# Hendrik1704/GPBayesTools-HIC

Hardware: AMD Instinct MI355X
Metric: MCMC steps/s x walkers (walker log-posterior evaluations per second, whole job) (higher is better)
Workload: dtype f64

## Files before the change

gpbayestools_hic_amd/csrc/gpb_api.hip:

```cpp
#include "gpb_internal.h"
#include <dlfcn.h>
#include <math.h>
#include <string.h>
#include <vector>
#include <mutex>
#include <condition_variable>

using namespace gpb;

namespace {

template <typename T>
int dev_alloc(gpb_ctx* ctx, T** p, int64_t count) {
    if (*p) {
        if (ctx->side_stream) GPB_HIP(hipStreamSynchronize(ctx->side_stream));
        pool_free(*p); *p = nullptr;
    }
    GPB_HIP(pool_malloc(reinterpret_cast<void**>(p), sizeof(T) * (size_t)(count > 0 ? count : 1)));
    return 0;
}
template <typename T>
void dev_free(T** p) {
    if (*p) { pool_free(*p); *p = nullptr; }
}
// ... 1008 lines not shown
}

extern "C" int gpb_ctx_option(gpb_ctx* ctx, int key, int value) {
    if (!ctx) return GPB_E_ARG;
#ifndef GPB_DEBUG_VARIANTS
    if ((key == 26 && value != 0) || (key == 32 && value != 0))
        GPB_FAIL(GPB_E_ARG, "gpb_ctx_option: this value selects a hook of the debug build only");
#endif
    switch (key) {
        case 0: if (value < -1 || value > 1) return GPB_E_ARG; ctx->force_xcd = value; break;
        case 4: if (value < 0 || value % 64) return GPB_E_ARG; ctx->chol_outer = value; break;
        case 5: if (value < 1 || value > 3) return GPB_E_ARG; ctx->resident_order = value; break;
        case 7: if (value < 0) return GPB_E_ARG; ctx->narrow_switch = value; break;
        case 8: if (value < 0) return GPB_E_ARG; ctx->mvn_wg_switch = value; break;
        case 9: if (value != 64 && value != 128) return GPB_E_ARG; ctx->chol_inner_tile = value; break;
        case 10: if (value < 0 || value > 1) return GPB_E_ARG; ctx->tile_priority = value; break;
        case 17: if (value < 0 || value > 1) return GPB_E_ARG; ctx->tri_skip = value; break;
        case 18:
            if (value < 0 || value > 2) return GPB_E_ARG;
            ctx->kcross_dot = value;
            if (ctx->have_theta) {
                const int rc = choose_forms(ctx);
                if (rc) return rc;
            }
            break;
        case 19: if (value < 0 || value > 64) return GPB_E_ARG; ctx->kcross_chunks = value; break;
        case 20: if (value < 1 || value > 2) return GPB_E_ARG; ctx->kcross_wpl = value; break;
        case 23: if (value < 0 || value > 1) return GPB_E_ARG; ctx->lowrank = value; break;
        case 22: if (value < 0) return GPB_E_ARG; ctx->mid_switch = value; break;
        case 11: if (value < 0 || value > 1) return GPB_E_ARG; ctx->fuse_finalize = value; break;
        case 12: if (value != 0 && value != 64 && value != 128) return GPB_E_ARG; ctx->trtri_tile = value; break;
        case 14: if (value != 0 && value != 64 && value != 128) return GPB_E_ARG; ctx->syrk_tile = value; break;
        case 25: if (value < 0 || value > 1) return GPB_E_ARG; ctx->chol_lookahead = value; break;
        case 26: if (value < 0 || value > 64) return GPB_E_ARG; ctx->sim_ranks = value; break;
        case 27: if (value < 0 || value > 1) return GPB_E_ARG; ctx->compact = value; break;
        case 28: if (value < 0 || value > 1) return GPB_E_ARG; ctx->tile_by_live = value; break;
        case 29: if (value < 0 || value > 2) return GPB_E_ARG; ctx->premark = value; break;
        case 30: if (value < 0 || value > 1) return GPB_E_ARG; ctx->fuse_accept_propose = value; break;
        case 32: if (value < 0 || value > 63) return GPB_E_ARG; ctx->sim_rank = value; break;
        case 36: if (value < 0 || value > 2) return GPB_E_ARG; ctx->balance_shards = value; break;
        case 40: if (value < 0 || value > 1) return GPB_E_ARG; ctx->chain_batch = value; break;
        case 42:
            if (value != 0 && value != 32 && value != 64 && value != 65 && value != 128) return GPB_E_ARG;
            ctx->force_tile = value;
            break;
        case 43: if (value < 0 || value > 1) return GPB_E_ARG; ctx->force_generic_mvn = value != 0; break;
        case 47: if (value < 0 || value > 2) return GPB_E_ARG; ctx->chol_pair = value; break;
        case 49: if (value < 0 || value > 1) return GPB_E_ARG; ctx->lr_split = value; break;
        case 50: if (value != 0 && value != 64 && value != 128) return GPB_E_ARG; ctx->kinv_tile = value; break;
        case 51:
            if (value < 0 || value > 3) return GPB_E_ARG;
            ctx->predict_sliced = value;
            break;
        case 44: if (value < 0) return GPB_E_ARG; ctx->tile_switch = value > 0 ? value : 960; break;
        case 33: if (value < 0) return GPB_E_ARG; ctx->tile_switch_c = value; break;
        case 34: if (value < 0) return GPB_E_ARG; ctx->mid_switch_c = value; break;
        case 35: if (value < 0) return GPB_E_ARG; ctx->narrow_switch_c = value; break;
        default: return GPB_E_ARG;
    }
    return 0;
}

extern "C" int gpb_profile_fit_piece(gpb_ctx* ctx, int piece) {
    if (!ctx) return GPB_E_ARG;
    if (!ctx->have_theta) GPB_FAIL(GPB_E_STATE, "gpb_profile_fit_piece before gpb_gp_set_theta");
    GPB_HIP(hipSetDevice(ctx->device));
    ctx->factored = false;
    switch (piece) {
        case 0: return launch_kmat(ctx);
        case 1: return launch_potrf(ctx);
        case 2: return launch_trtri(ctx);
        case 3: return launch_alpha(ctx);
        default: return GPB_E_ARG;
    }
}



extern "C" int gpb_profile_enable(gpb_ctx* ctx, int on) {
    if (!ctx) return GPB_E_ARG;
    ctx->profile = on != 0;
    return 0;
}

extern "C" int gpb_profile_read(gpb_ctx* ctx, int64_t* launches, double* total_ms, double* units) {
    if (!ctx || !launches || !total_ms || !units) return GPB_E_ARG;
    GPB_HIP(hipSetDevice(ctx->device));
    GPB_HIP(hipStreamSynchronize(ctx->stream));
    double ms = 0.0;
    for (auto& ev : ctx->prof_events) {
        float t = 0.f;
        GPB_HIP(hipEventElapsedTime(&t, ev.first, ev.second));
        ms += t;
        (void)hipEventDestroy(ev.first);
        (void)hipEventDestroy(ev.second);
    }
    if (ctx->prof_compacted) {
        unsigned long long live = 0;
        GPB_HIP(hipMemcpy(&live, ctx->rows_live, sizeof(live), hipMemcpyDeviceToHost));
        GPB_HIP(hipMemset(ctx->rows_live, 0, sizeof(live)));
        ctx->prof_units += (ctx->prof_gps > 0.0 ? ctx->prof_gps : (double)ctx->P) * (double)live;
        ctx->prof_compacted = false;
    }
    *launches = (int64_t)ctx->prof_events.size();
    *total_ms = ms;
    *units = ctx->prof_units;
// ... 42 lines not shown
```

gpbayestools_hic_amd/csrc/gpb_internal.h:

```cpp
#pragma once
#include <hip/hip_runtime.h>
#include <stdint.h>
#include <string>
#include <utility>
#include <vector>
#include "../../include/gpbayes.h"
#include "../../include/gpbayes_debug.h"

namespace gpb {

constexpr int NB = 64;
constexpr int WPAD = 128;
constexpr int KX_CHUNK = 64;
constexpr int MAX_D = 64;

inline int64_t round_up(int64_t a, int64_t b) { return (a + b - 1) / b * b; }
__host__ __device__ inline int64_t imin64(int64_t a, int64_t b) { return a < b ? a : b; }

}

struct GpSel {
    const int* map;
    const int* n;
    int N;
    int64_t x_stride, xm_stride;
    __device__ __forceinline__ int q(int a) const { return map ? map[a] : a; }
    __device__ __forceinline__ int64_t Nq(int qq) const { return n ? (int64_t)n[qq] : (int64_t)N; }
};

__host__ __device__ __forceinline__ int64_t pad_front(int64_t Np, int64_t N) { return ((Np - N) / 16) * 16; }

struct LoopGroup;
struct gpb_ctx {
    int device = 0;
    hipStream_t stream = nullptr;
    bool own_stream = false;
    std::string err;

    int64_t N = 0, Np = 0, d = 0, dpad = 0, P = 0;
    int kind = 0;
    double alpha_reg = 0.0;
    bool have_theta = false, factored = false;
    double* h_theta = nullptr;
    bool multi = false;
    int64_t Pstore = 0;
    int* gpN = nullptr;
    int* gpmap = nullptr;
    bool subset = false;
    std::vector<int> h_N;
    std::vector<int> h_map;
    GpSel sel() const {
        return GpSel{subset ? gpmap : nullptr, multi ? gpN : nullptr, (int)N, multi ? Np * dpad : 0, multi ? dpad : 0};
    }
    double* X = nullptr;
    double* Xsc = nullptr;
    double* xmean = nullptr;
    double* muS = nullptr;
    double* Xc = nullptr;
    double* dnorm = nullptr;
    std::vector<double> h_ext;
    std::vector<int> h_form;
    int* gpform = nullptr;
    int* kmtiles = nullptr;
    int n_diff = 0;
    double gram_limit = 1024.0;
    double* ls = nullptr;
    double* amp = nullptr;
    double* noise = nullptr;
    double* Z = nullptr;
    double* K = nullptr;
    double* Linv = nullptr;
    int predict_sliced = 3;
    int8_t* slA = nullptr;
    int8_t* slB = nullptr;
    double* sl_scale = nullptr;
    bool slA_valid = false;
    int slA_depth = 0;
    int64_t slB_cap = 0;
    int batch_sliced = 0;
    bool want_kst = false;
    double* T = nullptr;
    double* yv = nullptr;
    double* alpha = nullptr;
    double* apart = nullptr;
    int* info = nullptr;
    double* lmlbuf = nullptr;
    double* gpart = nullptr;
    int64_t gpart_cap = 0;

    int64_t Wcap = 0;
    int64_t last_W = 0;
    int64_t Wld = 0;
    double* Xs = nullptr;
    double* estd = nullptr;
    double* KsT = nullptr;
    double* mpart = nullptr;
    double* spart = nullptr;
    double* mean_pc = nullptr;
    double* var_pc = nullptr;
    unsigned long long* live_hint = nullptr;
    gpb_ctx* hint_from = nullptr;
    int fuse_accept_propose = 1;
    int balance_shards = 0;
    int* bal_ws = nullptr;
    int64_t bal_cap = 0;
    int sim_rank = 0;
    int tile_by_live = 1;
    int premark = 2;
    double* cmp_X = nullptr;
    int64_t cmp_X_cap = 0;
    int* cmp_idx = nullptr;
    int compact = 1;
    unsigned long long* rows_live = nullptr;
    bool prof_compacted = false;
    double* vbuf = nullptr;
    int64_t vbuf_cap = 0;
    double* gbuf = nullptr;
    int64_t gbuf_cap = 0;
    double* covbuf = nullptr;
    int64_t covbuf_cap = 0;
    double* out_stage = nullptr;
    int64_t out_cap = 0;
    int* cv_ws = nullptr;
    int64_t cv_cap = 0;
    std::vector<int> h_cv;
// ... 171 lines not shown
```

gpbayestools_hic_amd/csrc/gpb_sliced.hip:

```cpp
#include "gpb_internal.h"

namespace gpb {

typedef int v4i __attribute__((ext_vector_type(4)));
typedef int v16i __attribute__((ext_vector_type(16)));
typedef __attribute__((address_space(3))) void* sl_lds_ptr;

template <int D>
struct SlDig {
    static constexpr int LOW = D - 1, NLEV = 2 * D - 1 - LOW, BITS = 8 * D - 1;
    static constexpr unsigned long long HALF = 0x8080808080808080ull >> (64 - 8 * D);
};
constexpr int SL_DMAX = 7;
constexpr int64_t SL_NP_MAX = 16384;
constexpr int SL_BM = 128;
template <int D, int WTN>
struct SlGeo {
    static constexpr int BN = 64 * WTN;
    static constexpr int A_CHUNKS = D * 2 * (SL_BM / 64), B_CHUNKS = D * 2 * WTN, CHUNKS = A_CHUNKS + B_CHUNKS;
    static constexpr int STAGE = CHUNKS * 1024, NSTAGE = 3;
    static constexpr int LDS = NSTAGE * STAGE + SL_BM * 8;
    static constexpr int NPW = (CHUNKS + 7) / 8, REM = CHUNKS % 8;
};
constexpr int SL_RG = 8, SL_CG = 4;
constexpr double SL_RULE = 128.0;

template <int D>
__device__ __forceinline__ unsigned long long sl_digits(long long a) {
    return ((unsigned long long)a + SlDig<D>::HALF) ^ SlDig<D>::HALF;
}

__device__ __forceinline__ int sl_exponent(double m) {
    int ex;
    const double f = frexp(m, &ex);
    return f <= 0.99 ? ex : ex + 1;
}

__global__ __launch_bounds__(256) void k_sl_rowscale(const double* __restrict__ Linv, const double* __restrict__ amp,
                                                     double* __restrict__ rowscale, int* __restrict__ rowexp,
                                                     double* __restrict__ colscale, int64_t Np, int64_t Np128) {
    const int p = blockIdx.y, lane = threadIdx.x & 63;
    const int64_t j = (int64_t)blockIdx.x * 4 + (threadIdx.x >> 6);
    if (j >= Np128) return;
    double m = 0.0;
    if (j < Np) {
        const double* row = Linv + ((int64_t)p * Np + j) * Np;
        for (int64_t k = lane; k <= j; k += 64) m = fmax(m, fabs(row[k]));
#pragma unroll
        for (int o = 32; o > 0; o >>= 1) m = fmax(m, __shfl_xor(m, o));
    }
    if (lane == 0) {
        const int e = m > 0.0 ? sl_exponent(m) : 0;
        rowexp[(int64_t)p * Np128 + j] = e;
        rowscale[(int64_t)p * Np128 + j] = ldexp(1.0, e - 14);
        if (j == 0) colscale[p] = ldexp(1.0, sl_exponent(amp[p]));
    }
}

template <int D>
__global__ __launch_bounds__(256) void k_sl_slice_linv(const double* __restrict__ Linv, const int* __restrict__ rowexp,
                                                       int8_t* __restrict__ planes, int64_t Np, int64_t Np128) {
    const int p = blockIdx.z;
    const int64_t j = (int64_t)blockIdx.x * 256 + threadIdx.x, kb = blockIdx.y;
    if (j >= Np || kb * 16 > j) return;
    const double* src = Linv + ((int64_t)p * Np + j) * Np + kb * 16;
    const int e = rowexp[(int64_t)p * Np128 + j];
    unsigned long long dg[16];
#pragma unroll
    for (int i = 0; i < 16; ++i) {
        const double x = (kb * 16 + i <= j) ? src[i] : 0.0;
        dg[i] = sl_digits<D>(__double2ll_rn(ldexp(x, SlDig<D>::BITS - e)));
    }
    const int64_t plane = (Np / 16) * Np128 * 16;
    int8_t* dst = planes + (int64_t)p * D * plane + (kb * Np128 + j) * 16;
#pragma unroll
    for (int t = 0; t < D; ++t) {
// ... 23 lines not shown
        const int t = cb / (2 * per), q = (cb / per) & 1, h = cb % per;
        const int64_t ld = is_a ? Np128 : Wld, off = is_a ? mb : nb;
        const int8_t* plane = is_a ? Ap + t * a_plane : Bp + t * b_plane;
        const int8_t* src = plane + ((kb0 + q) * ld + off + 64 * h + lane) * 16;
        __builtin_amdgcn_global_load_lds((const void*)src, (sl_lds_ptr)(base + ch * 1024), 16, 0, 0);
    }
}

template <int N>
__device__ __forceinline__ void sl_wait_vm() { asm volatile("s_waitcnt vmcnt(%0)" ::"n"(N) : "memory"); }

template <int D, int WTN>
__device__ __forceinline__ void sl_wait_stage(bool more, bool full_count) {
    typedef SlGeo<D, WTN> G;
    if (!more) sl_wait_vm<0>();
    else if (full_count) sl_wait_vm<G::NPW>();
    else sl_wait_vm<G::NPW - 1>();
}

template <int D, int WTN>
__device__ __forceinline__ void sl_mma_step(const char* lds, int buf, int wm, int wn, int lane, v16i (&acc)[SlDig<D>::NLEV][WTN]) {
    typedef SlGeo<D, WTN> G;
    constexpr int LOW = SlDig<D>::LOW;
    const char* base = lds + buf * G::STAGE;
    const int q = lane >> 5, r = lane & 31;
    v4i a[D];
#pragma unroll
    for (int t = 0; t < D; ++t) a[t] = *reinterpret_cast<const v4i*>(base + ((t * 2 + q) * SL_BM + wm * 32 + r) * 16);
#pragma unroll
    for (int j = 0; j < WTN; ++j) {
        v4i b[D];
#pragma unroll
        for (int t = 0; t < D; ++t)
            b[t] = *reinterpret_cast<const v4i*>(base + G::A_CHUNKS * 1024 + ((t * 2 + q) * G::BN + wn * 32 * WTN + 32 * j + r) * 16);
#pragma unroll
        for (int tb = 0; tb < D; ++tb)
#pragma unroll
            for (int ta = 0; ta < D; ++ta) {
                if (ta + tb < LOW) continue;
                acc[ta + tb - LOW][j] = __builtin_amdgcn_mfma_i32_32x32x32_i8(a[ta], b[tb], acc[ta + tb - LOW][j], 0, 0, 0);
            }
    }
}

struct SlGP {
    const int8_t *A, *B;
    const double *rowscale, *colscale;
    double* spart;
    int P, p;
};
constexpr int SL_MAX_GP = GPB_MAX_MULTI_GP;
struct SlTable { SlGP gp[SL_MAX_GP]; };

template <int D, int WTN, bool MULTI>
__device__ __forceinline__ void predict_sliced_body(const SlGP& G0, const SlTable* __restrict__ tab, int64_t Np, int64_t Np128, int64_t Wld,
                                                    int P, int nI, int nW, int kskip, const int* __restrict__ nrows) {
    typedef SlGeo<D, WTN> G;
    constexpr int NLEV = SlDig<D>::NLEV;
    extern __shared__ __attribute__((aligned(16))) char lds[];
    if (nrows) nW = (*nrows + G::BN - 1) / G::BN;
    const int nG = (nI + SL_RG - 1) / SL_RG, nWG = (nW + SL_CG - 1) / SL_CG;
    const unsigned label = blockIdx.x & 7u, m = blockIdx.x >> 3;
    const unsigned sb = (m / (SL_RG * SL_CG)) * 8u + label, local = m % (SL_RG * SL_CG);
    if (sb >= (unsigned)(nG * P * nWG)) return;
    const int g = (int)(sb / (unsigned)(P * nWG)), rem = (int)(sb % (unsigned)(P * nWG));
    const int pg = rem / nWG, wg = rem % nWG;
    const SlGP gp = MULTI ? tab->gp[pg] : G0;
    const int p = MULTI ? gp.p : pg;
    const int8_t* __restrict__ A = gp.A;
    const int8_t* __restrict__ B = gp.B;
    const double* __restrict__ rowscale = gp.rowscale;
    const double* __restrict__ colscale = gp.colscale;
    double* __restrict__ spart = gp.spart;
    const int Pc = MULTI ? gp.P : P;
    const int ib = (nG - 1 - g) * SL_RG + (SL_RG - 1 - (int)(local / SL_CG)), wt = wg * SL_CG + (int)(local % SL_CG);
    if (ib >= nI || wt >= nW) return;
    const int tid = threadIdx.x, lane = tid & 63;
    const int wave = __builtin_amdgcn_readfirstlane(tid >> 6);
    const int wm = wave >> 1, wn = wave & 1;
    const int64_t mb = (int64_t)ib * SL_BM, nb = (int64_t)wt * G::BN;
    const bool fullc = G::REM == 0 || wave < G::REM;
    const int64_t a_plane = (Np / 16) * Np128 * 16, b_plane = (Np / 16) * Wld * 16;
    const int8_t* Ap = A + (int64_t)p * D * a_plane;
    const int8_t* Bp = B + (int64_t)p * D * b_plane;
    double* rs = reinterpret_cast<double*>(lds + G::NSTAGE * G::STAGE);
    if (tid < SL_BM) rs[tid] = rowscale[(int64_t)p * Np128 + mb + tid];
    const int64_t k_end = imin64(mb + SL_BM, Np);
    const int64_t ks = (kskip / 32) * 32;
    const int64_t k_begin = ks <= mb ? ks : 0;
    const int nsteps = (int)((k_end - k_begin) / 32);
    const int64_t kb_first = k_begin / 16;
    v16i acc[NLEV][WTN];
#pragma unroll
    for (int l = 0; l < NLEV; ++l)
#pragma unroll
        for (int j = 0; j < WTN; ++j)
#pragma unroll
            for (int r = 0; r < 16; ++r) acc[l][j][r] = 0;
    sl_dma_stage<D, WTN>(lds, 0, Ap, Bp, a_plane, b_plane, Np128, Wld, mb, nb, kb_first, wave, lane);
    if (nsteps > 1) sl_dma_stage<D, WTN>(lds, 1, Ap, Bp, a_plane, b_plane, Np128, Wld, mb, nb, kb_first + 2, wave, lane);
    for (int s = 0; s < nsteps; ++s) {
        asm volatile("s_waitcnt lgkmcnt(0)" ::: "memory");
        sl_wait_stage<D, WTN>(s + 1 < nsteps, fullc);
        __builtin_amdgcn_s_barrier();
        sl_mma_step<D, WTN>(lds, s % 3, wm, wn, lane, acc);
        if (s + 2 < nsteps)
            sl_dma_stage<D, WTN>(lds, (s + 2) % 3, Ap, Bp, a_plane, b_plane, Np128, Wld, mb, nb, kb_first + 2 * (int64_t)(s + 2), wave, lane);
    }
    asm volatile("s_waitcnt lgkmcnt(0)" ::: "memory");
    __builtin_amdgcn_s_barrier();
    const double cs = colscale[p];
    double* hand = reinterpret_cast<double*>(lds);
    double sums[WTN];
#pragma unroll
    for (int j = 0; j < WTN; ++j) {
        double sum = 0.0;
#pragma unroll
        for (int r = 0; r < 16; ++r) {
            double t = (double)acc[0][j][r];
#pragma unroll
            for (int l = 1; l < NLEV; ++l) t = fma(t, 1.0 / 256.0, (double)acc[l][j][r]);
            const int row = wm * 32 + (r & 3) + 8 * (r >> 2) + 4 * (lane >> 5);
            const double v = t * rs[row] * cs;
            sum = fma(v, v, sum);
        }
        sum += __shfl_xor(sum, 32);
        sums[j] = sum;
        if ((wm & 1) && lane < 32) hand[(wave * WTN + j) * 32 + lane] = sum;
    }
    __syncthreads();
    const int64_t blk = (int64_t)ib * 2 + (wm >> 1);
    if (!(wm & 1) && lane < 32 && blk * 64 < Np) {
#pragma unroll
        for (int j = 0; j < WTN; ++j)
            spart[(blk * Pc + p) * Wld + nb + wn * 32 * WTN + 32 * j + lane] = sums[j] + hand[((wave + 2) * WTN + j) * 32 + lane];
    }
}

template <int D, int WTN>
__global__ __launch_bounds__(512, 2) void k_predict_sliced(const SlGP gp, int64_t Np, int64_t Np128, int64_t Wld, int P, int nI, int nW,
                                                           int kskip, const int* __restrict__ nrows) {
    predict_sliced_body<D, WTN, false>(gp, nullptr, Np, Np128, Wld, P, nI, nW, kskip, nrows);
}

template <int D, int WTN>
__global__ __launch_bounds__(512, 2) void k_predict_sliced_multi(const SlTable tab, int64_t Np, int64_t Np128, int64_t Wld, int P, int nI,
                                                                 int nW, int kskip, const int* __restrict__ nrows) {
    predict_sliced_body<D, WTN, true>(tab.gp[0], &tab, Np, Np128, Wld, P, nI, nW, kskip, nrows);
}

int sliced_applies(const gpb_ctx* ctx) {
    if (!ctx->predict_sliced || ctx->multi || !ctx->h_theta || !ctx->have_theta) return 0;
    if (ctx->tile_trace) return 0;
    if (ctx->Np > SL_NP_MAX) return 0;
    if (ctx->predict_sliced == 3) return 7;
    if (ctx->predict_sliced == 2) return 6;
    const int64_t stride = ctx->d + 2;
    for (int64_t p = 0; p < ctx->P; ++p) {
        const double lc = ctx->h_theta[p * stride], ln = ctx->h_theta[p * stride + ctx->d + 1];
        if (!(1.0 + exp(lc - ln) <= SL_RULE)) return 0;
    }
    return 6;
}

void sliced_free(gpb_ctx* ctx) {
    if (ctx->slA) { pool_free(ctx->slA); ctx->slA = nullptr; }
    if (ctx->slB) { pool_free(ctx->slB); ctx->slB = nullptr; }
    if (ctx->sl_scale) { pool_free(ctx->sl_scale); ctx->sl_scale = nullptr; }
    ctx->slA_valid = false;
    ctx->slA_depth = 0;
    ctx->slB_cap = 0;
}

const double* sliced_colscale(const gpb_ctx* ctx) {
    return reinterpret_cast<const double*>(ctx->sl_scale) + ctx->P * round_up(ctx->Np, 128);
}

int sliced_prepare(gpb_ctx* ctx, int depth) {
    if (depth != 6 && depth != 7) GPB_FAIL(GPB_E_STATE, "gpb: internal: sliced_prepare at a depth other than 6 or 7");
    const int64_t Np = ctx->Np, Np128 = round_up(Np, 128), P = ctx->P;
    const size_t a_bytes = (size_t)P * SL_DMAX * (size_t)Np * (size_t)Np128;
    if (!ctx->slA) {
        GPB_HIP(pool_malloc_t(&ctx->slA, a_bytes));
        GPB_HIP(hipMemsetAsync(ctx->slA, 0, a_bytes, ctx->stream));
        GPB_HIP(pool_malloc_t(&ctx->sl_scale, sizeof(double) * (size_t)(P * Np128 + P) + sizeof(int) * (size_t)(P * Np128)));
        ctx->slA_valid = false;
    }
    double* rowscale = reinterpret_cast<double*>(ctx->sl_scale);
    double* colscale = rowscale + P * Np128;
    int* rowexp = reinterpret_cast<int*>(colscale + P);
    if (!ctx->slA_valid || ctx->slA_depth != depth) {
        hipLaunchKernelGGL(k_sl_rowscale, dim3((unsigned)((Np128 + 3) / 4), (unsigned)P), dim3(256), 0, ctx->stream, ctx->Linv,
                           ctx->amp, rowscale, rowexp, colscale, Np, Np128);
        const dim3 grid((unsigned)((Np + 255) / 256), (unsigned)(Np / 16), (unsigned)P);
        if (depth == 7)
            hipLaunchKernelGGL(k_sl_slice_linv<7>, grid, dim3(256), 0, ctx->stream, ctx->Linv, rowexp, ctx->slA, Np, Np128);
        else
            hipLaunchKernelGGL(k_sl_slice_linv<6>, grid, dim3(256), 0, ctx->stream, ctx->Linv, rowexp, ctx->slA, Np, Np128);
        ctx->slA_valid = true;
        ctx->slA_depth = depth;
    }
    if (ctx->slB_cap < ctx->Wcap || !ctx->slB) {
        if (ctx->slB) { GPB_HIP(hipStreamSynchronize(ctx->stream)); pool_free(ctx->slB); ctx->slB = nullptr; }
        GPB_HIP(pool_malloc_t(&ctx->slB, (size_t)P * SL_DMAX * (size_t)Np * (size_t)ctx->Wcap));
        ctx->slB_cap = ctx->Wcap;
    }
    GPB_HIP(hipGetLastError());
    return 0;
}

int sliced_read_kstar(gpb_ctx* ctx, int64_t p, int64_t pad, int64_t N, int64_t W, double* out) {
    const int D = ctx->batch_sliced;
    if (D != 6 && D != 7) GPB_FAIL(GPB_E_STATE, "gpb: internal: sliced_read_kstar without a sliced batch");
    const int64_t Np = ctx->Np, Wld = ctx->Wld, plane = (Np / 16) * Wld * 16;
    std::vector<int8_t> h((size_t)(D * plane));
    double cs = 0.0;
    GPB_HIP(hipStreamSynchronize(ctx->stream));
    GPB_HIP(hipMemcpy(h.data(), ctx->slB + p * D * plane, (size_t)(D * plane), hipMemcpyDeviceToHost));
    GPB_HIP(hipMemcpy(&cs, sliced_colscale(ctx) + p, sizeof(double), hipMemcpyDeviceToHost));
    for (int64_t n = 0; n < N; ++n)
        for (int64_t w = 0; w < W; ++w) {
            const int64_t k = pad + n;
            long long a = 0;
            for (int t = D - 1; t >= 0; --t) a = a * 256 + (long long)h[(size_t)(t * plane + ((k / 16) * Wld + w) * 16 + k % 16)];
            out[n * W + w] = ldexp((double)a, -(8 * D - 1)) * cs;
        }
    return 0;
}

static int sliced_wtn(const gpb_ctx* ctx, int depth, int64_t gps, int nI, int64_t W, const int* nrows_dev) {
    if (depth == 7) return 1;
    const int64_t Wsel = imin64(ctx->Wld, live_rows_estimate(ctx, W, nrows_dev, ctx->Wld));
    const int64_t tiles128 = gps * nI * ((Wsel + 127) / 128);
    int wtn = tiles128 >= 3 * (int64_t)ctx->num_cu ? 2 : 1;
    if (ctx->force_tile == 128) wtn = 2;
    if (ctx->force_tile == 64 || ctx->force_tile == 32 || ctx->force_tile == 65) wtn = 1;
    return wtn;
}

template <int D, int WTN, bool MULTI, class Arg>
static int sliced_launch(gpb_ctx* ctx, const Arg& arg, int64_t Np, int64_t Np128, int64_t Wld, int G, int nI, int kskip,
                         const int* nrows_dev) {
    typedef SlGeo<D, WTN> Geo;
    const int nW = (int)(Wld / Geo::BN);
    const int nG = (nI + SL_RG - 1) / SL_RG, nWG = (nW + SL_CG - 1) / SL_CG;
    const int64_t nSB = (int64_t)nG * G * nWG;
    const unsigned grid = (unsigned)(((nSB + 7) / 8) * 8 * SL_RG * SL_CG);
    if constexpr (MULTI) {
        GPB_HIP(hipFuncSetAttribute((const void*)k_predict_sliced_multi<D, WTN>, hipFuncAttributeMaxDynamicSharedMemorySize, Geo::LDS));
        hipLaunchKernelGGL((k_predict_sliced_multi<D, WTN>), dim3(grid), dim3(512), Geo::LDS, ctx->stream, arg, Np, Np128, Wld, G, nI, nW,
                           kskip, nrows_dev);
    } else {
        GPB_HIP(hipFuncSetAttribute((const void*)k_predict_sliced<D, WTN>, hipFuncAttributeMaxDynamicSharedMemorySize, Geo::LDS));
        hipLaunchKernelGGL((k_predict_sliced<D, WTN>), dim3(grid), dim3(512), Geo::LDS, ctx->stream, arg, Np, Np128, Wld, G, nI, nW,
                           kskip, nrows_dev);
    }
    return 0;
}

template <bool MULTI, class Arg>
static int sliced_dispatch(gpb_ctx* ctx, int depth, int wtn, const Arg& arg, int64_t Np, int64_t Np128, int64_t Wld, int G, int nI,
                           int kskip, const int* nrows_dev) {
    if (depth == 7) return sliced_launch<7, 1, MULTI>(ctx, arg, Np, Np128, Wld, G, nI, kskip, nrows_dev);
    if (wtn == 2) return sliced_launch<6, 2, MULTI>(ctx, arg, Np, Np128, Wld, G, nI, kskip, nrows_dev);
    return sliced_launch<6, 1, MULTI>(ctx, arg, Np, Np128, Wld, G, nI, kskip, nrows_dev);
}

int launch_vsq_sliced(gpb_ctx* ctx, int64_t W, const int* nrows_dev, int kskip) {
    const int64_t Np = ctx->Np, Np128 = round_up(Np, 128), P = ctx->P, Wld = ctx->Wld;
    const int depth = ctx->batch_sliced;
    if (!ctx->slA || !ctx->slA_valid || !ctx->slB || ctx->slA_depth != depth)
        GPB_FAIL(GPB_E_STATE, "gpb: internal: launch_vsq_sliced before sliced_prepare");
    const double* rowscale = reinterpret_cast<const double*>(ctx->sl_scale);
    const double* colscale = rowscale + P * Np128;
    const int nI = (int)(Np128 / SL_BM);
    const int wtn = sliced_wtn(ctx, depth, P, nI, W, nrows_dev);
    const SlGP gp{ctx->slA, ctx->slB, rowscale, colscale, ctx->spart, (int)P, 0};
    return sliced_dispatch<false>(ctx, depth, wtn, gp, Np, Np128, Wld, (int)P, nI, kskip, nrows_dev);
}

int launch_vsq_sliced_multi(gpb_ctx* const* ctxs, int E, int64_t W, const int* nrows_dev, int kskip) {
    gpb_ctx* ctx = ctxs[0];
    const int64_t Np = ctx->Np, Np128 = round_up(Np, 128), Wld = ctx->Wld;
    const int depth = ctx->batch_sliced;
    SlTable tab;
    int G = 0;
    for (int e = 0; e < E; ++e) {
        gpb_ctx* c = ctxs[e];
        if (!c->slA || !c->slA_valid || !c->slB || c->Np != Np || c->Wld != Wld || c->batch_sliced != depth || c->slA_depth != depth)
            GPB_FAIL(GPB_E_STATE, "gpb: internal: launch_vsq_sliced_multi over a context that is not prepared");
        const double* rowscale = reinterpret_cast<const double*>(c->sl_scale);
        const double* colscale = rowscale + c->P * Np128;
        for (int p = 0; p < (int)c->P; ++p, ++G) {
            if (G >= SL_MAX_GP) GPB_FAIL(GPB_E_STATE, "gpb: internal: launch_vsq_sliced_multi: too many GPs for one table");
            tab.gp[G] = SlGP{c->slA, c->slB, rowscale, colscale, c->spart, (int)c->P, p};
        }
    }
    const int nI = (int)(Np128 / SL_BM);
    const int wtn = sliced_wtn(ctx, depth, G, nI, W, nrows_dev);
    return sliced_dispatch<true>(ctx, depth, wtn, tab, Np, Np128, Wld, G, nI, kskip, nrows_dev);
}

}
```

gpbayestools_hic_amd/engine.py:

```python
import ctypes as C
import itertools
import os

import numpy as np

from . import _native as nat

KERNEL_IDS = {"RBF": 0, "Matern": 1, "Matern15": 1, "Matern25": 2}
MODE_PCA, MODE_NO_PCA, MODE_EXPDIAG, MODE_NO_PCA_EXPDIAG = 0, 1, 2, 3


class NotPositiveDefinite(np.linalg.LinAlgError):
    pass


def _is_torch(x):
    return hasattr(x, "data_ptr") and hasattr(x, "is_cuda")


_SERIAL = itertools.count(1)

PREDICT_SLICED_DEFAULT = 3
_PREDICT_SLICED_ENV = {"0": 0, "fp64": 0, "1": 1, "int8": 1, "2": 2, "3": 3, "fp64-int8": 3}

# ... 427 lines not shown
        return rec[:n.value]

    def dist_available(self):
        return self.lib.gpb_dist_available() == 1

    def dist_uid(self):
        uid = np.zeros(128, dtype=np.uint8)
        self._ck(self.lib.gpb_dist_uid(nat.ptr(uid)))
        return uid.tobytes()

    def dist_init(self, rank, nranks, uid):
        buf = np.frombuffer(bytes(uid), dtype=np.uint8).copy()
        if buf.size != 128:
            raise ValueError("uid must be the 128 bytes of dist_uid()")
        self._ck(self.lib.gpb_dist_init(self.h, int(rank), int(nranks), nat.ptr(buf)))
        self._dist_world = int(nranks)

    def dist_allgather(self, send, recv):
        self._track_stream()
        n = send.numel()
        self._dev(send, (n,), "send")
        self._dev(recv, (n * getattr(self, "_dist_world", 0),), "recv")
        self._ck(self.lib.gpb_dist_allgather(self.h, nat.VP(send.data_ptr()), nat.VP(recv.data_ptr()), n))
        return recv

    def dist_finalize(self):
        self._ck(self.lib.gpb_dist_finalize(self.h))
        self._dist_world = 0

    def test_gemm(self, A, B, mode=0, tile=128):
        A, B = nat.f64(A), nat.f64(B)
        if mode == 0:
            M, K = A.shape; N = B.shape[1]
        elif mode == 1:
            M, K = A.shape; N = B.shape[0]
        else:
            K, M = A.shape; N = B.shape[1]
        Cm = np.empty((M, N))
        self._ck(self.lib.gpb_test_gemm(self.h, M, N, K, nat.ptr(A), nat.ptr(B), nat.ptr(Cm),
                                        mode | (4 if tile == 64 else 0)))
        return Cm

    def force_tile(self, tile=0, switch_tiles=0):
        self.tune("force_tile", int(tile))
        if switch_tiles > 0:
            self.tune("tile_switch", int(switch_tiles))

    def tune(self, key, value):
        k = {"xcd": 0, "chol_outer": 4, "resident": 5, "narrow_switch": 7, "mvn_wg_switch": 8, "chol_inner_tile": 9,
             "tile_priority": 10, "fuse_finalize": 11, "trtri_tile": 12, "syrk_tile": 14, "tri_skip": 17, "kcross_dot": 18,
             "kcross_chunks": 19, "kcross_wpl": 20, "mid_switch": 22, "lowrank": 23, "chol_lookahead": 25, "sim_ranks": 26,
             "compact": 27, "tile_by_live": 28, "premark": 29, "fuse_accept_propose": 30, "sim_rank": 32, "tile_switch_c": 33,
             "mid_switch_c": 34, "narrow_switch_c": 35, "balance_shards": 36, "chain_batch": 40, "force_tile": 42, "generic_mvn": 43,
             "tile_switch": 44, "chol_pair": 47, "lr_split": 49, "kinv_tile": 50, "predict_sliced": 51}[key]
        self._ck(self.lib.gpb_ctx_option(self.h, k, int(value)))
        if k == 51:
            self.predict_sliced = int(value)

    @property
    def has_variants(self):
        return self.lib.gpb_debug_has_variants() == 1

    def fit_piece(self, piece):
        self._ck(self.lib.gpb_profile_fit_piece(self.h, {"kmat": 0, "potrf": 1, "trtri": 2, "alpha": 3}[piece]))

    def force_generic_mvn(self, on=True):
        self.tune("generic_mvn", 1 if on else 0)

    def profile(self, on=True):
        self._ck(self.lib.gpb_profile_enable(self.h, 1 if on else 0))

    def profile_read(self):
        n, ms, u = C.c_int64(0), C.c_double(0.0), C.c_double(0.0)
        self._ck(self.lib.gpb_profile_read(self.h, C.byref(n), C.byref(ms), C.byref(u)))
        return n.value, ms.value, u.value

    def probe_fp64(self, mode):
        out = C.c_double(0.0)
        self._ck(self.lib.gpb_probe_fp64(self.h, int(mode), C.byref(out)))
        return out.value
```

Baseline: 1.597 million.

## Add persistent work-queue form of the int8-sliced predict kernel with cross-tile prefetch

Adds a persistent variant of the sliced int8 MFMA predict kernel. A grid about the size of the CU count pulls tiles from per-XCD atomic queues and prefetches the next tile's first stages and rowscale while it reduces and stores the current one. This is meant to cut launch and tail overhead and hide the per-tile pipeline fill. In exchange it adds atomics, extra LDS for double-buffered scales, and a queue reset that relies on the last workgroup. It is on by default (sliced_persist=1) whenever there are more tiles than slots.

```diff
diff --git a/gpbayestools_hic_amd/csrc/gpb_api.hip b/gpbayestools_hic_amd/csrc/gpb_api.hip
--- a/gpbayestools_hic_amd/csrc/gpb_api.hip
+++ b/gpbayestools_hic_amd/csrc/gpb_api.hip
@@ -1084,6 +1084,10 @@
             if (value < 0 || value > 3) return GPB_E_ARG;
             ctx->predict_sliced = value;
             break;
+        case 52:
+            if (value < 0 || (value > 1 && value < 8) || value > 4096) return GPB_E_ARG;
+            ctx->sliced_persist = (int)value;
+            break;
         case 44: if (value < 0) return GPB_E_ARG; ctx->tile_switch = value > 0 ? value : 960; break;
         case 33: if (value < 0) return GPB_E_ARG; ctx->tile_switch_c = value; break;
         case 34: if (value < 0) return GPB_E_ARG; ctx->mid_switch_c = value; break;
diff --git a/gpbayestools_hic_amd/csrc/gpb_internal.h b/gpbayestools_hic_amd/csrc/gpb_internal.h
--- a/gpbayestools_hic_amd/csrc/gpb_internal.h
+++ b/gpbayestools_hic_amd/csrc/gpb_internal.h
@@ -71,6 +71,7 @@
     double* K = nullptr;
     double* Linv = nullptr;
     int predict_sliced = 3;
+    int sliced_persist = 1;
     int8_t* slA = nullptr;
     int8_t* slB = nullptr;
     double* sl_scale = nullptr;
diff --git a/gpbayestools_hic_amd/csrc/gpb_sliced.hip b/gpbayestools_hic_amd/csrc/gpb_sliced.hip
--- a/gpbayestools_hic_amd/csrc/gpb_sliced.hip
+++ b/gpbayestools_hic_amd/csrc/gpb_sliced.hip
@@ -21,7 +21,14 @@
     static constexpr int STAGE = CHUNKS * 1024, NSTAGE = 3;
     static constexpr int LDS = NSTAGE * STAGE + SL_BM * 8;
     static constexpr int NPW = (CHUNKS + 7) / 8, REM = CHUNKS % 8;
+    static constexpr int HAND_OFF = NSTAGE * STAGE, HAND = 8 * WTN * 32 * 8;
+    static constexpr int RS_OFF = HAND_OFF + HAND, TICKET_OFF = RS_OFF + 2 * SL_BM * 8;
+    static constexpr int CS_OFF = TICKET_OFF + 16, LDS_PERSIST = CS_OFF + 16;
 };
+static_assert(SlGeo<7, 1>::LDS_PERSIST <= 160 * 1024 && SlGeo<6, 1>::LDS_PERSIST <= 160 * 1024 && SlGeo<6, 2>::LDS_PERSIST <= 160 * 1024,
+              "the persistent form's LDS must fit a CU");
+static_assert(SlGeo<7, 1>::LDS_PERSIST > 80 * 1024 && SlGeo<6, 1>::LDS_PERSIST > 80 * 1024 && SlGeo<6, 2>::LDS_PERSIST > 80 * 1024,
+              "the persistent form counts on ONE workgroup per CU");
 constexpr int SL_RG = 8, SL_CG = 4;
 constexpr double SL_RULE = 128.0;
 
@@ -151,88 +158,244 @@
 constexpr int SL_MAX_GP = GPB_MAX_MULTI_GP;
 struct SlTable { SlGP gp[SL_MAX_GP]; };
 
+struct SlTile {
+    const int8_t *Ap, *Bp;
+    const double *rowscale, *colscale;
+    double* spart;
+    int Pc, p, ib;
+    int64_t mb, nb, kb_first;
+    int nsteps;
+};
+
+template <int D, int WTN, bool MULTI>
+__device__ __forceinline__ bool sl_tile_decode(SlTile& T, unsigned sb, unsigned local, const SlGP& G0, const SlTable* __restrict__ tab,
+                                               int64_t Np, int64_t Np128, int64_t Wld, int P, int nI, int nW, int nG, int nWG, int kskip) {
+    typedef SlGeo<D, WTN> G;
+    const int g = (int)(sb / (unsigned)(P * nWG)), rem = (int)(sb % (unsigned)(P * nWG));
+    const int pg = rem / nWG, wg = rem % nWG;
+    const int ib = (nG - 1 - g) * SL_RG + (SL_RG - 1 - (int)(local / SL_CG)), wt = wg * SL_CG + (int)(local % SL_CG);
+    if (ib >= nI || wt >= nW) return false;
+    const SlGP gp = MULTI ? tab->gp[pg] : G0;
+    const int p = MULTI ? gp.p : pg;
+    const int64_t a_plane = (Np / 16) * Np128 * 16, b_plane = (Np / 16) * Wld * 16;
+    T.Ap = gp.A + (int64_t)p * D * a_plane;
+    T.Bp = gp.B + (int64_t)p * D * b_plane;
+    T.mb = (int64_t)ib * SL_BM;
+    T.nb = (int64_t)wt * G::BN;
+    T.rowscale = gp.rowscale + (int64_t)p * Np128 + T.mb;
+    T.colscale = gp.colscale + p;
+    T.spart = gp.spart;
+    T.Pc = MULTI ? gp.P : P;
+    T.p = p;
+    T.ib = ib;
+    const int64_t k_end = imin64(T.mb + SL_BM, Np);
+    const int64_t ks = (kskip / 32) * 32;
+    const int64_t k_begin = ks <= T.mb ? ks : 0;
+    T.nsteps = (int)((k_end - k_begin) / 32);
+    T.kb_first = k_begin / 16;
+    return true;
+}
+
+template <int D, int WTN>
+__device__ __forceinline__ void sl_tile_prologue(char* lds, const SlTile& T, int64_t Np, int64_t Np128, int64_t Wld, int wave, int lane) {
+    const int64_t a_plane = (Np / 16) * Np128 * 16, b_plane = (Np / 16) * Wld * 16;
+    sl_dma_stage<D, WTN>(lds, 0, T.Ap, T.Bp, a_plane, b_plane, Np128, Wld, T.mb, T.nb, T.kb_first, wave, lane);
+    if (T.nsteps > 1) sl_dma_stage<D, WTN>(lds, 1, T.Ap, T.Bp, a_plane, b_plane, Np128, Wld, T.mb, T.nb, T.kb_first + 2, wave, lane);
+}
+
+template <int D, int WTN>
+__device__ __forceinline__ void sl_tile_kloop(char* lds, const SlTile& T, int64_t Np, int64_t Np128, int64_t Wld, int wave, int lane,
+                                              v16i (&acc)[SlDig<D>::NLEV][WTN]) {
+    typedef SlGeo<D, WTN> G;
+    const int wm = wave >> 1, wn = wave & 1;
+    const bool fullc = G::REM == 0 || wave < G::REM;
+    const int64_t a_plane = (Np / 16) * Np128 * 16, b_plane = (Np / 16) * Wld * 16;
+    const int nsteps = T.nsteps;
+    for (int s = 0; s < nsteps; ++s) {
+        asm volatile("s_waitcnt lgkmcnt(0)" ::: "memory");
+        sl_wait_stage<D, WTN>(s + 1 < nsteps, fullc);
+        __builtin_amdgcn_s_barrier();
+        sl_mma_step<D, WTN>(lds, s % 3, wm, wn, lane, acc);
+        if (s + 2 < nsteps)
+            sl_dma_stage<D, WTN>(lds, (s + 2) % 3, T.Ap, T.Bp, a_plane, b_plane, Np128, Wld, T.mb, T.nb, T.kb_first + 2 * (int64_t)(s + 2), wave,
+                                 lane);
+    }
+}
+
+__device__ __forceinline__ void sl_tile_close() {
+    asm volatile("s_waitcnt lgkmcnt(0)" ::: "memory");
+    __builtin_amdgcn_s_barrier();
+}
+
+template <int D, int WTN>
+__device__ __forceinline__ void sl_tile_sums(const v16i (&acc)[SlDig<D>::NLEV][WTN], const double* rs, double cs, double* hand, int wave,
+                                             int lane, double (&sums)[WTN]) {
+    constexpr int NLEV = SlDig<D>::NLEV;
+    const int wm = wave >> 1;
+#pragma unroll
+    for (int j = 0; j < WTN; ++j) {
+        double sum = 0.0;
+#pragma unroll
+        for (int r = 0; r < 16; ++r) {
+            double t = (double)acc[0][j][r];
+#pragma unroll
+            for (int l = 1; l < NLEV; ++l) t = fma(t, 1.0 / 256.0, (double)acc[l][j][r]);
+            const int row = wm * 32 + (r & 3) + 8 * (r >> 2) + 4 * (lane >> 5);
+            const double v = t * rs[row] * cs;
+            sum = fma(v, v, sum);
+        }
+        sum += __shfl_xor(sum, 32);
+        sums[j] = sum;
+        if ((wm & 1) && lane < 32) hand[(wave * WTN + j) * 32 + lane] = sum;
+    }
+}
+
+template <int D, int WTN>
+__device__ __forceinline__ void sl_tile_store(const SlTile& T, int64_t Np, int64_t Wld, const double* hand, int wave, int lane,
+                                              const double (&sums)[WTN]) {
+    const int wm = wave >> 1, wn = wave & 1;
+    const int64_t blk = (int64_t)T.ib * 2 + (wm >> 1);
+    if (!(wm & 1) && lane < 32 && blk * 64 < Np) {
+#pragma unroll
+        for (int j = 0; j < WTN; ++j)
+            T.spart[(blk * T.Pc + T.p) * Wld + T.nb + wn * 32 * WTN + 32 * j + lane] = sums[j] + hand[((wave + 2) * WTN + j) * 32 + lane];
+    }
+}
+
+template <int D, int WTN>
+__device__ __forceinline__ void sl_zero(v16i (&acc)[SlDig<D>::NLEV][WTN]) {
+#pragma unroll
+    for (int l = 0; l < SlDig<D>::NLEV; ++l)
+#pragma unroll
+        for (int j = 0; j < WTN; ++j)
+#pragma unroll
+            for (int r = 0; r < 16; ++r) acc[l][j][r] = 0;
+}
+
 template <int D, int WTN, bool MULTI>
 __device__ __forceinline__ void predict_sliced_body(const SlGP& G0, const SlTable* __restrict__ tab, int64_t Np, int64_t Np128, int64_t Wld,
                                                     int P, int nI, int nW, int kskip, const int* __restrict__ nrows) {
     typedef SlGeo<D, WTN> G;
-    constexpr int NLEV = SlDig<D>::NLEV;
     extern __shared__ __attribute__((aligned(16))) char lds[];
     if (nrows) nW = (*nrows + G::BN - 1) / G::BN;
     const int nG = (nI + SL_RG - 1) / SL_RG, nWG = (nW + SL_CG - 1) / SL_CG;
     const unsigned label = blockIdx.x & 7u, m = blockIdx.x >> 3;
     const unsigned sb = (m / (SL_RG * SL_CG)) * 8u + label, local = m % (SL_RG * SL_CG);
     if (sb >= (unsigned)(nG * P * nWG)) return;
-    const int g = (int)(sb / (unsigned)(P * nWG)), rem = (int)(sb % (unsigned)(P * nWG));
-    const int pg = rem / nWG, wg = rem % nWG;
-    const SlGP gp = MULTI ? tab->gp[pg] : G0;
-    const int p = MULTI ? gp.p : pg;
-    const int8_t* __restrict__ A = gp.A;
-    const int8_t* __restrict__ B = gp.B;
-    const double* __restrict__ rowscale = gp.rowscale;
-    const double* __restrict__ colscale = gp.colscale;
-    double* __restrict__ spart = gp.spart;
-    const int Pc = MULTI ? gp.P : P;
-    const int ib = (nG - 1 - g) * SL_RG + (SL_RG - 1 - (int)(local / SL_CG)), wt = wg * SL_CG + (int)(local % SL_CG);
-    if (ib >= nI || wt >= nW) return;
+    SlTile T;
+    if (!sl_tile_decode<D, WTN, MULTI>(T, sb, local, G0, tab, Np, Np128, Wld, P, nI, nW, nG, nWG, kskip)) return;
     const int tid = threadIdx.x, lane = tid & 63;
     const int wave = __builtin_amdgcn_readfirstlane(tid >> 6);
-    const int wm = wave >> 1, wn = wave & 1;
-    const int64_t mb = (int64_t)ib * SL_BM, nb = (int64_t)wt * G::BN;
-    const bool fullc = G::REM == 0 || wave < G::REM;
-    const int64_t a_plane = (Np / 16) * Np128 * 16, b_plane = (Np / 16) * Wld * 16;
-    const int8_t* Ap = A + (int64_t)p * D * a_plane;
-    const int8_t* Bp = B + (int64_t)p * D * b_plane;
     double* rs = reinterpret_cast<double*>(lds + G::NSTAGE * G::STAGE);
-    if (tid < SL_BM) rs[tid] = rowscale[(int64_t)p * Np128 + mb + tid];
-    const int64_t k_end = imin64(mb + SL_BM, Np);
-    const int64_t ks = (kskip / 32) * 32;
-    const int64_t k_begin = ks <= mb ? ks : 0;
-    const int nsteps = (int)((k_end - k_begin) / 32);
-    const int64_t kb_first = k_begin / 16;
-    v16i acc[NLEV][WTN];
-#pragma unroll
-    for (int l = 0; l < NLEV; ++l)
-#pragma unroll
-        for (int j = 0; j < WTN; ++j)
-#pragma unroll
-            for (int r = 0; r < 16; ++r) acc[l][j][r] = 0;
-    sl_dma_stage<D, WTN>(lds, 0, Ap, Bp, a_plane, b_plane, Np128, Wld, mb, nb, kb_first, wave, lane);
-    if (nsteps > 1) sl_dma_stage<D, WTN>(lds, 1, Ap, Bp, a_plane, b_plane, Np128, Wld, mb, nb, kb_first + 2, wave, lane);
-    for (int s = 0; s < nsteps; ++s) {
-        asm volatile("s_waitcnt lgkmcnt(0)" ::: "memory");
-        sl_wait_stage<D, WTN>(s + 1 < nsteps, fullc);
-        __builtin_amdgcn_s_barrier();
-        sl_mma_step<D, WTN>(lds, s % 3, wm, wn, lane, acc);
-        if (s + 2 < nsteps)
-            sl_dma_stage<D, WTN>(lds, (s + 2) % 3, Ap, Bp, a_plane, b_plane, Np128, Wld, mb, nb, kb_first + 2 * (int64_t)(s + 2), wave, lane);
-    }
-    asm volatile("s_waitcnt lgkmcnt(0)" ::: "memory");
-    __builtin_amdgcn_s_barrier();
-    const double cs = colscale[p];
+    if (tid < SL_BM) rs[tid] = T.rowscale[tid];
+    v16i acc[SlDig<D>::NLEV][WTN];
+    sl_zero<D, WTN>(acc);
+    sl_tile_prologue<D, WTN>(lds, T, Np, Np128, Wld, wave, lane);
+    sl_tile_kloop<D, WTN>(lds, T, Np, Np128, Wld, wave, lane, acc);
+    sl_tile_close();
     double* hand = reinterpret_cast<double*>(lds);
     double sums[WTN];
-#pragma unroll
-    for (int j = 0; j < WTN; ++j) {
-        double sum = 0.0;
-#pragma unroll
-        for (int r = 0; r < 16; ++r) {
-            double t = (double)acc[0][j][r];
-#pragma unroll
-            for (int l = 1; l < NLEV; ++l) t = fma(t, 1.0 / 256.0, (double)acc[l][j][r]);
-            const int row = wm * 32 + (r & 3) + 8 * (r >> 2) + 4 * (lane >> 5);
-            const double v = t * rs[row] * cs;
-            sum = fma(v, v, sum);
-        }
-        sum += __shfl_xor(sum, 32);
-        sums[j] = sum;
-        if ((wm & 1) && lane < 32) hand[(wave * WTN + j) * 32 + lane] = sum;
-    }
+    sl_tile_sums<D, WTN>(acc, rs, *T.colscale, hand, wave, lane, sums);
     __syncthreads();
-    const int64_t blk = (int64_t)ib * 2 + (wm >> 1);
-    if (!(wm & 1) && lane < 32 && blk * 64 < Np) {
-#pragma unroll
-        for (int j = 0; j < WTN; ++j)
-            spart[(blk * Pc + p) * Wld + nb + wn * 32 * WTN + 32 * j + lane] = sums[j] + hand[((wave + 2) * WTN + j) * 32 + lane];
+    sl_tile_store<D, WTN>(T, Np, Wld, hand, wave, lane, sums);
+}
+
+template <int D, int WTN, bool MULTI>
+__device__ __forceinline__ void predict_sliced_persist_body(const SlGP& G0, const SlTable* __restrict__ tab, int64_t Np, int64_t Np128,
+                                                            int64_t Wld, int P, int nI, int nW, int kskip, const int* __restrict__ nrows,
+                                                            unsigned* __restrict__ queue) {
+    typedef SlGeo<D, WTN> G;
+    extern __shared__ __attribute__((aligned(16))) char lds[];
+    if (nrows) nW = (*nrows + G::BN - 1) / G::BN;
+    const int nG = (nI + SL_RG - 1) / SL_RG, nWG = (nW + SL_CG - 1) / SL_CG;
+    const unsigned nSB = (unsigned)(nG * P * nWG);
+    const unsigned label = blockIdx.x & 7u;
+    const int tid = threadIdx.x, lane = tid & 63;
+    const int wave = __builtin_amdgcn_readfirstlane(tid >> 6);
+    double* hand = reinterpret_cast<double*>(lds + G::HAND_OFF);
+    double* rs = reinterpret_cast<double*>(lds + G::RS_OFF);
+    unsigned* s_ticket = reinterpret_cast<unsigned*>(lds + G::TICKET_OFF);
+    double* cs2 = reinterpret_cast<double*>(lds + G::CS_OFF);
+    unsigned* q = queue + label * 16u;
+
+    auto next_live = [&](unsigned m, SlTile& T) -> bool {
+        for (;;) {
+            const unsigned sb = (m / (SL_RG * SL_CG)) * 8u + label;
+            if (sb >= nSB) return false;
+            if (sl_tile_decode<D, WTN, MULTI>(T, sb, m % (SL_RG * SL_CG), G0, tab, Np, Np128, Wld, P, nI, nW, nG, nWG, kskip)) return true;
+            __syncthreads();
+            if (tid == 0) s_ticket[1] = atomicAdd(q, 1u);
+            __syncthreads();
+            m = (unsigned)__builtin_amdgcn_readfirstlane((int)s_ticket[1]);
+        }
+    };
+    auto prefetch = [&](const SlTile& T, int rb) {
+        if (wave == 7)
+            __builtin_amdgcn_global_load_lds((const void*)(T.rowscale + 2 * lane), (sl_lds_ptr)(lds + G::RS_OFF + rb * SL_BM * 8), 16, 0, 0);
+        sl_tile_prologue<D, WTN>(lds, T, Np, Np128, Wld, wave, lane);
+    };
+
+    if (tid == 0) s_ticket[1] = atomicAdd(q, 1u);
+    __syncthreads();
+    int rb = 0;
+    bool have;
+    {
+        SlTile first;
+        have = next_live((unsigned)__builtin_amdgcn_readfirstlane((int)s_ticket[1]), first);
+        __syncthreads();
+        if (have) {
+            prefetch(first, rb);
+            if (tid == 0) {
+                cs2[rb] = *first.colscale;
+                s_ticket[0] = s_ticket[1];
+                s_ticket[1] = atomicAdd(q, 1u);
+            }
+        }
+        sl_wait_vm<0>();
+        __syncthreads();
+    }
+    while (have) {
+        SlTile cur;
+        const unsigned m = (unsigned)__builtin_amdgcn_readfirstlane((int)s_ticket[0]);
+        (void)sl_tile_decode<D, WTN, MULTI>(cur, (m / (SL_RG * SL_CG)) * 8u + label, m % (SL_RG * SL_CG), G0, tab, Np, Np128, Wld, P, nI, nW,
+                                            nG, nWG, kskip);
+        v16i acc[SlDig<D>::NLEV][WTN];
+        sl_zero<D, WTN>(acc);
+        sl_tile_kloop<D, WTN>(lds, cur, Np, Np128, Wld, wave, lane, acc);
+        sl_tile_close();
+        unsigned ahead;
+        double cs_next;
+        bool drawer;
+        {
+            SlTile nxt;
+            have = next_live((unsigned)__builtin_amdgcn_readfirstlane((int)s_ticket[1]), nxt);
+            drawer = have && tid == 0;
+            if (have) prefetch(nxt, rb ^ 1);
+            if (drawer) {
+                cs_next = *nxt.colscale;
+                ahead = atomicInc(q, 0xffffffffu);
+            }
+        }
+        double sums[WTN];
+        sl_tile_sums<D, WTN>(acc, rs + rb * SL_BM, cs2[rb], hand, wave, lane, sums);
+        asm volatile("s_waitcnt lgkmcnt(0)" ::: "memory");
+        __builtin_amdgcn_s_barrier();
+        sl_tile_store<D, WTN>(cur, Np, Wld, hand, wave, lane, sums);
+        if (drawer) {
+            s_ticket[0] = s_ticket[1];
+            s_ticket[1] = ahead;
+            cs2[rb ^ 1] = cs_next;
+        }
+        sl_wait_vm<0>();
+        asm volatile("s_waitcnt lgkmcnt(0)" ::: "memory");
+        __builtin_amdgcn_s_barrier();
+        rb ^= 1;
+    }
+    if (tid == 0) {
+        if (atomicAdd(&queue[128], 1u) == gridDim.x - 1) {
+            for (int i = 0; i < 8; ++i) queue[i * 16] = 0u;
+            queue[128] = 0u;
+        }
     }
 }
 
@@ -246,6 +409,20 @@
 __global__ __launch_bounds__(512, 2) void k_predict_sliced_multi(const SlTable tab, int64_t Np, int64_t Np128, int64_t Wld, int P, int nI,
                                                                  int nW, int kskip, const int* __restrict__ nrows) {
     predict_sliced_body<D, WTN, true>(tab.gp[0], &tab, Np, Np128, Wld, P, nI, nW, kskip, nrows);
+}
+
+template <int D, int WTN>
+__global__ __launch_bounds__(512, 2) void k_predict_sliced_persist(const SlGP gp, int64_t Np, int64_t Np128, int64_t Wld, int P, int nI,
+                                                                   int nW, int kskip, const int* __restrict__ nrows,
+                                                                   unsigned* __restrict__ queue) {
+    predict_sliced_persist_body<D, WTN, false>(gp, nullptr, Np, Np128, Wld, P, nI, nW, kskip, nrows, queue);
+}
+
+template <int D, int WTN>
+__global__ __launch_bounds__(512, 2) void k_predict_sliced_persist_multi(const SlTable tab, int64_t Np, int64_t Np128, int64_t Wld, int P,
+                                                                         int nI, int nW, int kskip, const int* __restrict__ nrows,
+                                                                         unsigned* __restrict__ queue) {
+    predict_sliced_persist_body<D, WTN, true>(tab.gp[0], &tab, Np, Np128, Wld, P, nI, nW, kskip, nrows, queue);
 }
 
 int sliced_applies(const gpb_ctx* ctx) {
@@ -337,13 +514,36 @@
     return wtn;
 }
 
+static unsigned sliced_persist_grid(const gpb_ctx* ctx, int bn, int64_t gps, int nI, int64_t W, const int* nrows_dev) {
+    if (ctx->sliced_persist == 0) return 0u;
+    if (ctx->sliced_persist >= 8) return (unsigned)((ctx->sliced_persist + 7) / 8 * 8);
+    const unsigned slots = (unsigned)((ctx->num_cu + 7) / 8 * 8);
+    const int64_t Wsel = imin64(ctx->Wld, live_rows_estimate(ctx, W, nrows_dev, ctx->Wld));
+    const int64_t tiles = gps * nI * ((Wsel + bn - 1) / bn);
+    return tiles > (int64_t)slots ? slots : 0u;
+}
+
 template <int D, int WTN, bool MULTI, class Arg>
-static int sliced_launch(gpb_ctx* ctx, const Arg& arg, int64_t Np, int64_t Np128, int64_t Wld, int G, int nI, int kskip,
+static int sliced_launch(gpb_ctx* ctx, const Arg& arg, int64_t Np, int64_t Np128, int64_t Wld, int G, int nI, int kskip, int64_t W,
                          const int* nrows_dev) {
     typedef SlGeo<D, WTN> Geo;
     const int nW = (int)(Wld / Geo::BN);
     const int nG = (nI + SL_RG - 1) / SL_RG, nWG = (nW + SL_CG - 1) / SL_CG;
     const int64_t nSB = (int64_t)nG * G * nWG;
+    if (const unsigned pgrid = sliced_persist_grid(ctx, Geo::BN, G, nI, W, nrows_dev)) {
+        if constexpr (MULTI) {
+            GPB_HIP(hipFuncSetAttribute((const void*)k_predict_sliced_persist_multi<D, WTN>, hipFuncAttributeMaxDynamicSharedMemorySize,
+                                        Geo::LDS_PERSIST));
+            hipLaunchKernelGGL((k_predict_sliced_persist_multi<D, WTN>), dim3(pgrid), dim3(512), Geo::LDS_PERSIST, ctx->stream, arg, Np, Np128,
+                               Wld, G, nI, nW, kskip, nrows_dev, ctx->tile_counter);
+        } else {
+            GPB_HIP(hipFuncSetAttribute((const void*)k_predict_sliced_persist<D, WTN>, hipFuncAttributeMaxDynamicSharedMemorySize,
+                                        Geo::LDS_PERSIST));
+            hipLaunchKernelGGL((k_predict_sliced_persist<D, WTN>), dim3(pgrid), dim3(512), Geo::LDS_PERSIST, ctx->stream, arg, Np, Np128, Wld, G,
+                               nI, nW, kskip, nrows_dev, ctx->tile_counter);
+        }
+        return 0;
+    }
     const unsigned grid = (unsigned)(((nSB + 7) / 8) * 8 * SL_RG * SL_CG);
     if constexpr (MULTI) {
         GPB_HIP(hipFuncSetAttribute((const void*)k_predict_sliced_multi<D, WTN>, hipFuncAttributeMaxDynamicSharedMemorySize, Geo::LDS));
@@ -359,10 +559,10 @@
 
 template <bool MULTI, class Arg>
 static int sliced_dispatch(gpb_ctx* ctx, int depth, int wtn, const Arg& arg, int64_t Np, int64_t Np128, int64_t Wld, int G, int nI,
-                           int kskip, const int* nrows_dev) {
-    if (depth == 7) return sliced_launch<7, 1, MULTI>(ctx, arg, Np, Np128, Wld, G, nI, kskip, nrows_dev);
-    if (wtn == 2) return sliced_launch<6, 2, MULTI>(ctx, arg, Np, Np128, Wld, G, nI, kskip, nrows_dev);
-    return sliced_launch<6, 1, MULTI>(ctx, arg, Np, Np128, Wld, G, nI, kskip, nrows_dev);
+                           int kskip, int64_t W, const int* nrows_dev) {
+    if (depth == 7) return sliced_launch<7, 1, MULTI>(ctx, arg, Np, Np128, Wld, G, nI, kskip, W, nrows_dev);
+    if (wtn == 2) return sliced_launch<6, 2, MULTI>(ctx, arg, Np, Np128, Wld, G, nI, kskip, W, nrows_dev);
+    return sliced_launch<6, 1, MULTI>(ctx, arg, Np, Np128, Wld, G, nI, kskip, W, nrows_dev);
 }
 
 int launch_vsq_sliced(gpb_ctx* ctx, int64_t W, const int* nrows_dev, int kskip) {
@@ -375,7 +575,7 @@
     const int nI = (int)(Np128 / SL_BM);
     const int wtn = sliced_wtn(ctx, depth, P, nI, W, nrows_dev);
     const SlGP gp{ctx->slA, ctx->slB, rowscale, colscale, ctx->spart, (int)P, 0};
-    return sliced_dispatch<false>(ctx, depth, wtn, gp, Np, Np128, Wld, (int)P, nI, kskip, nrows_dev);
+    return sliced_dispatch<false>(ctx, depth, wtn, gp, Np, Np128, Wld, (int)P, nI, kskip, W, nrows_dev);
 }
 
 int launch_vsq_sliced_multi(gpb_ctx* const* ctxs, int E, int64_t W, const int* nrows_dev, int kskip) {
@@ -397,7 +597,7 @@
     }
     const int nI = (int)(Np128 / SL_BM);
     const int wtn = sliced_wtn(ctx, depth, G, nI, W, nrows_dev);
-    return sliced_dispatch<true>(ctx, depth, wtn, tab, Np, Np128, Wld, G, nI, kskip, nrows_dev);
-}
-
-}
+    return sliced_dispatch<true>(ctx, depth, wtn, tab, Np, Np128, Wld, G, nI, kskip, W, nrows_dev);
+}
+
+}
diff --git a/gpbayestools_hic_amd/engine.py b/gpbayestools_hic_amd/engine.py
--- a/gpbayestools_hic_amd/engine.py
+++ b/gpbayestools_hic_amd/engine.py
@@ -503,7 +503,7 @@
              "kcross_chunks": 19, "kcross_wpl": 20, "mid_switch": 22, "lowrank": 23, "chol_lookahead": 25, "sim_ranks": 26,
              "compact": 27, "tile_by_live": 28, "premark": 29, "fuse_accept_propose": 30, "sim_rank": 32, "tile_switch_c": 33,
              "mid_switch_c": 34, "narrow_switch_c": 35, "balance_shards": 36, "chain_batch": 40, "force_tile": 42, "generic_mvn": 43,
-             "tile_switch": 44, "chol_pair": 47, "lr_split": 49, "kinv_tile": 50, "predict_sliced": 51}[key]
+             "tile_switch": 44, "chol_pair": 47, "lr_split": 49, "kinv_tile": 50, "predict_sliced": 51, "sliced_persist": 52}[key]
         self._ck(self.lib.gpb_ctx_option(self.h, k, int(value)))
         if k == 51:
             self.predict_sliced = int(value)
```

Result: no change. 1.594 million (-0.1%).
